# NICTA/revrand

Measured on AMD Instinct MI355X. Metric: feature-rows/sec (Phi + PhiT Phi + PhiT y) at N=10M D=32 F=4096, higher is better.
Workload: dtype f32; 1 GPU; RandomRBF nbases=2048 (F=4096), D=32, N=10000000 f32, features + MFMA Gram, rows sharded over 1 GPU(s); rows_per_gpu=10000000, device=(gfx950:sramecc+:xnack-), gram_engine=f32

## Files before the change

revrand_amd/csrc/rr_rff.hip:

```cpp
#include "rr_syrk_args.h"
#include <algorithm>
#include <map>
#include <mutex>
#include <type_traits>




__device__ __forceinline__ void sincos_rev(float t, float &s, float &c) {
    const float f = t - __builtin_rintf(t);
    s = __builtin_amdgcn_sinf(f);
    c = __builtin_amdgcn_cosf(f);
}

__device__ __forceinline__ void sincos_rev(double t, double &s, double &c) { rr_sincos_rev_f64(t, s, c); }
typedef double doublex4 __attribute__((ext_vector_type(4)));

template <int DMAX, bool GUARD, typename TX, typename TC>
__device__ __forceinline__ TC project_row(const TX *__restrict__ xr, int d, const TC (&w)[DMAX]) {
    TC z = 0;
#pragma unroll
    for (int i = 0; i < DMAX; ++i) {
        if (!GUARD || i < d) z = fma((TC)xr[i], w[i], z);
    }
    return z;
}

template <int DMAX, typename TC>
__device__ __forceinline__ void load_w(TC (&w)[DMAX], const TC *__restrict__ Ws, int npad, int f) {
#pragma unroll
    for (int i = 0; i < DMAX; ++i) w[i] = Ws[(size_t)i * npad + f];
}

constexpr int RR_XS_ROWS = 16;
template <int DMAX, typename TX, typename TC>
__device__ __forceinline__ void stage_x_rows(TC (*xs)[DMAX], const TX *__restrict__ X, int64_t rb, int64_t rvalid, int64_t ldx) {
    for (int e = threadIdx.x; e < RR_XS_ROWS * DMAX; e += 256) {
        const int rr = e / DMAX, i = e % DMAX;
        xs[rr][i] = (rb + rr < rvalid) ? (TC)X[(rb + rr) * ldx + i] : (TC)0;
    }
}
template <int DMAX, typename TC>
__device__ __forceinline__ TC project_lds(const TC *__restrict__ xr, const TC (&w)[DMAX]) {
    TC z0 = 0, z1 = 0, z2 = 0, z3 = 0;
#pragma unroll
    for (int i = 0; i < DMAX; i += 4) {
        z0 = fma(xr[i], w[i], z0);
        z1 = fma(xr[i + 1], w[i + 1], z1);
        z2 = fma(xr[i + 2], w[i + 2], z2);
        z3 = fma(xr[i + 3], w[i + 3], z3);
    }
    return (z0 + z1) + (z2 + z3);
}

template <int DMAX, typename TX, typename TC, typename TO>
__global__ void __launch_bounds__(256)
rr_rff_transform_kernel(const TX *__restrict__ X, int64_t N, int64_t ldx, const TC *__restrict__ Ws,
                        int n, int npad, TO *__restrict__ Phi, int64_t ldphi, TC scale,
                        int rows_per_block) {
    const int f = blockIdx.x * 256 + threadIdx.x;
    const bool fvalid = f < n;
    TC w[DMAX];
    load_w<DMAX, TC>(w, Ws, npad, fvalid ? f : 0);
    const int64_t r0 = (int64_t)blockIdx.y * rows_per_block;
    int64_t r1 = r0 + rows_per_block;
    if (r1 > N) r1 = N;
    if constexpr (sizeof(TC) == 8 && DMAX >= 8) {
        __shared__ TC xs[RR_XS_ROWS][DMAX];
        for (int64_t rb = r0; rb < r1; rb += RR_XS_ROWS) {
            __syncthreads();
            stage_x_rows<DMAX, TX, TC>(xs, X, rb, r1, ldx);
            __syncthreads();
            const int nr = (int)(r1 - rb < RR_XS_ROWS ? r1 - rb : RR_XS_ROWS);
            for (int rr = 0; rr < nr; ++rr) {
                TC s, c;
                sincos_rev(project_lds<DMAX, TC>(xs[rr], w), s, c);
                if (fvalid) {
                    TO *o = Phi + (rb + rr) * ldphi;
                    o[f] = (TO)(c * scale);
                    o[n + f] = (TO)(s * scale);
                }
            }
        }
        return;
    }
    for (int64_t r = r0; r < r1; ++r) {
        const TC t = project_row<DMAX, false, TX, TC>(X + r * ldx, DMAX, w);
// ... 879 lines not shown
            RR_PAIRD(4, o0, o1) RR_PAIRD(5, o1, o0) RR_PAIRD(6, o0, o1) RR_PAIRD(7, o1, o0)
            __syncthreads();
        }
    }

    const int64_t F = p.F;
    const int hi = lane >> 5;
#pragma unroll
    for (int e = 0; e < NB; ++e) {
        const int64_t gc = ca + 32 * bj[e] + (lane & 31);
#pragma unroll
        for (int k = 0; k < 16; ++k) {
            const int64_t gr = ca + 32 * bi[e] + (k & 3) + 8 * (k >> 2) + 4 * hi;
            if (gr <= gc) rr_syrk_out(p, ks, gr, gc, acc[e][k]);
        }
    }
    (void)F;
}
#undef RR_PAIRD

__global__ void __launch_bounds__(GR_THREADS, 2)
rr_syrk_f32_diag_kernel(const SyrkArgs p) {
    __shared__ float lds[2 * GR_KB * GR_TC];
    const int lane = threadIdx.x & 63;
    const int wave = __builtin_amdgcn_readfirstlane(threadIdx.x >> 6);
    if (wave < 4)
        syrk_diag_body<5>(p, lds, wave, lane);
    else
        syrk_diag_body<4>(p, lds, wave, lane);
}

typedef float floatx4 __attribute__((ext_vector_type(4)));

template <int OFF>
__device__ __forceinline__ float lds_read_b32_off(unsigned addr) {
    float r;
    asm volatile("ds_read_b32 %0, %1 offset:%2" : "=v"(r) : "v"(addr), "i"(OFF));
    return r;
}

template <int NB, int ED>
struct KOpsD16 {
    float2v a[NB], b[NB];
    float x0, x1;
    template <int P>
    __device__ __forceinline__ void load(const unsigned (&abase)[NB], const unsigned (&bbase)[NB], unsigned xbase) {
#pragma unroll
        for (int e = 0; e < NB; ++e)
            if (e != ED) a[e] = lds_read2st64<16 * P, 16 * P + 8>(abase[e]);
#pragma unroll
        for (int e = 0; e < NB; ++e)
            if (e != ED) b[e] = lds_read2st64<16 * P, 16 * P + 8>(bbase[e]);
        x0 = lds_read_b32_off<4096 * P>(xbase);
        x1 = lds_read_b32_off<4096 * P + 64>(xbase);
    }
};

template <int NB, int ED, int FIRST, int LAST>
__device__ __forceinline__ void gram_mfma_d16(const KOpsD16<NB, ED> &o, floatx16 (&acc)[NB], floatx4 (&dd)[3]) {
#pragma unroll
    for (int q = FIRST; q < LAST; ++q) {
        if (q < NB - 1 || q >= NB + 2) {
            const int s_ = q < NB - 1 ? 0 : 1;
            const int r_ = q < NB - 1 ? q : q - (NB + 2);
            const int e = r_ < ED ? r_ : r_ + 1;
            acc[e] = __builtin_amdgcn_mfma_f32_32x32x2f32(o.a[e][s_], o.b[e][s_], acc[e], 0, 0, 0);
        } else {
            const int t = q - (NB - 1);
            dd[t] = __builtin_amdgcn_mfma_f32_16x16x4f32(t == 2 ? o.x1 : o.x0, t == 0 ? o.x0 : o.x1, dd[t], 0, 0, 0);
        }
    }
}

#define RR_PAIRD16(P, CUR, NXT)                                \
    lds_wait();                                                \
    __builtin_amdgcn_sched_barrier(0);                         \
    gram_mfma_d16<NB, ED, 0, 1>(CUR, acc, dd);                 \
    __builtin_amdgcn_sched_barrier(0);                         \
    if ((P) + 1 < KB / 4) NXT.template load<((P) + 1) & (KB / 4 - 1)>(abase, bbase, xbase); \
    __builtin_amdgcn_sched_barrier(0);                         \
    gram_mfma_d16<NB, ED, 1, 2 * NB + 1>(CUR, acc, dd);        \
    __builtin_amdgcn_sched_barrier(0);

template <int NB, int ED, int KB>
__device__ __forceinline__ void syrk_diag16_body(const SyrkArgs &p, float *lds, int wave, int lane, const unsigned bid) {
    const int ta = bid % p.nb;
    const int ks = bid / p.nb;
    const int ca = ta * GR_TC;
    const int64_t row_begin = (int64_t)ks * p.rows_per_split;
    int64_t row_end = row_begin + p.rows_per_split;
    if (row_end > p.rows) row_end = p.rows;

    const unsigned lds0 = (unsigned)(size_t)(__attribute__((address_space(3))) float *)lds;
    const unsigned lane_off = 4u * ((lane >> 5) * GR_TC + (lane & 31));
    int bi[NB], bj[NB];
#pragma unroll
    for (int e = 0; e < NB; ++e) {
        bi[e] = RR_DIAG_I[wave][e];
        bj[e] = RR_DIAG_J[wave][e];
    }
    RR_DEV_ASSERT(bi[ED] == bj[ED]);
    const unsigned lane_off16 = 4u * ((lane >> 4) * GR_TC + 32 * bi[ED] + (lane & 15));
    floatx16 acc[NB];
    floatx4 dd[3];
#pragma unroll
    for (int e = 0; e < NB; ++e)
#pragma unroll
        for (int k = 0; k < 16; ++k) acc[e][k] = 0.f;
#pragma unroll
    for (int t = 0; t < 3; ++t) dd[t] = floatx4{0.f, 0.f, 0.f, 0.f};

    const unsigned voff = 16u * lane, ldp4 = (unsigned)p.ldp * 4u;
    auto dma_tile = [&](float *buf, int64_t kb0) {
        RR_DEV_ASSERT(kb0 + KB <= p.rows && ca + GR_TC <= p.ldp && p.rows % KB == 0 && p.rows_per_split % KB == 0);
        const rr_rsrc_t ra = rr_make_rsrc(p.P + kb0 * p.ldp + ca, 0x7fffffffu);
#pragma unroll
        for (int k = 0; k < KB / 8; ++k) {
            const int lr = (KB / 8) * wave + k;
            __builtin_amdgcn_raw_ptr_buffer_load_lds(ra, (lptr_t)(buf + lr * GR_TC), 16, voff, (unsigned)lr * ldp4, 0, 0);
        }
    };

    const int64_t nkb = (row_end - row_begin) / KB;
    if (nkb > 0) {
        dma_tile(lds, row_begin);
        __syncthreads();
        for (int64_t kb = 0; kb < nkb; ++kb) {
            const int cbuf = (int)(kb & 1);
            const int slot = p.spread ? rr_dma_slot(wave, p.spread) : 0;
            auto dma_next = [&]() {
                if (kb + 1 < nkb) dma_tile(lds + (cbuf ^ 1) * (KB * GR_TC), row_begin + (kb + 1) * KB);
            };
            if (slot == 0) dma_next();
            unsigned abase[NB], bbase[NB];
#pragma unroll
            for (int e = 0; e < NB; ++e) {
                abase[e] = lds0 + cbuf * (4u * KB * GR_TC) + lane_off + 128u * bi[e];
                bbase[e] = lds0 + cbuf * (4u * KB * GR_TC) + lane_off + 128u * bj[e];
            }
            const unsigned xbase = lds0 + cbuf * (4u * KB * GR_TC) + lane_off16;
            KOpsD16<NB, ED> o0, o1;
            o0.template load<0>(abase, bbase, xbase);
            RR_PAIRD16(0, o0, o1)
            if (slot == 1) dma_next();
            RR_PAIRD16(1, o1, o0)
            if (slot == 2) dma_next();
            RR_PAIRD16(2, o0, o1)
            if (slot == 3) dma_next();
            RR_PAIRD16(3, o1, o0)
            RR_PAIRD16(4, o0, o1) RR_PAIRD16(5, o1, o0) RR_PAIRD16(6, o0, o1) RR_PAIRD16(7, o1, o0)
            if constexpr (KB == 64) {
                RR_PAIRD16(8, o0, o1) RR_PAIRD16(9, o1, o0) RR_PAIRD16(10, o0, o1) RR_PAIRD16(11, o1, o0)
                RR_PAIRD16(12, o0, o1) RR_PAIRD16(13, o1, o0) RR_PAIRD16(14, o0, o1) RR_PAIRD16(15, o1, o0)
            }
            __syncthreads();
        }
    }

    const int hi = lane >> 5;
#pragma unroll
    for (int e = 0; e < NB; ++e) {
        if (e == ED) continue;
        const int64_t gc = ca + 32 * bj[e] + (lane & 31);
#pragma unroll
        for (int k = 0; k < 16; ++k) {
            const int64_t gr = ca + 32 * bi[e] + (k & 3) + 8 * (k >> 2) + 4 * hi;
            if (gr <= gc) rr_syrk_out(p, ks, gr, gc, acc[e][k]);
        }
    }
#pragma unroll
    for (int t = 0; t < 3; ++t) {
        const int64_t gc = ca + 32 * bi[ED] + (t >= 1 ? 16 : 0) + (lane & 15);
#pragma unroll
        for (int k = 0; k < 4; ++k) {
            const int64_t gr = ca + 32 * bi[ED] + (t == 2 ? 16 : 0) + 4 * (lane >> 4) + k;
            if (gr <= gc) rr_syrk_out(p, ks, gr, gc, dd[t][k]);
        }
    }
}
#undef RR_PAIRD16

template <int KB>
__device__ __forceinline__ void syrk_diag16_dispatch(const SyrkArgs &p, float *lds, const unsigned bid) {
    const int lane = threadIdx.x & 63;
    const int wave = __builtin_amdgcn_readfirstlane(threadIdx.x >> 6);
    switch (wave) {
        case 0: case 1: case 2: case 3: syrk_diag16_body<5, 0, KB>(p, lds, wave, lane, bid); break;
        case 4: syrk_diag16_body<4, 3, KB>(p, lds, wave, lane, bid); break;
        case 5: syrk_diag16_body<4, 2, KB>(p, lds, wave, lane, bid); break;
        case 6: syrk_diag16_body<4, 1, KB>(p, lds, wave, lane, bid); break;
        default: syrk_diag16_body<4, 0, KB>(p, lds, wave, lane, bid); break;
    }
}

template <int KB>
__global__ void __launch_bounds__(GR_THREADS, 2)
rr_syrk_f32_diag16_kernel(const SyrkArgs p) {
    __shared__ float lds[2 * KB * GR_TC];
    syrk_diag16_dispatch<KB>(p, lds, blockIdx.x);
}

constexpr int GS_TC = 128, GS_KB = 32, GS_LD = 2 * GS_TC, GS_THREADS = 256;

__global__ void __launch_bounds__(GS_THREADS, 2)
rr_syrk_f32_small_kernel(const SyrkArgs p) {
    __shared__ __attribute__((aligned(16))) float lds[2][GS_KB * GS_LD];
    const int tid = threadIdx.x, lane = tid & 63, wave = tid >> 6, wr = wave >> 1, wc = wave & 1;
    const int nb = (int)(p.ldp / GS_TC);
    const int64_t ks = blockIdx.x / p.ntiles;
    int t = (int)(blockIdx.x % p.ntiles), ta = 0;
    while (t >= nb - ta) {
        t -= nb - ta;
        ++ta;
    }
    const int tb = ta + t;
    const int64_t ca = (int64_t)ta * GS_TC, cb = (int64_t)tb * GS_TC;
    const int64_t r0 = ks * p.rows_per_split;
    int64_t r1 = r0 + p.rows_per_split;
    if (r1 > p.rows) r1 = p.rows;
    const int nkb = (int)((r1 - r0 + GS_KB - 1) / GS_KB);
    floatx16 acc[2][2];
#pragma unroll
    for (int i = 0; i < 2; ++i)
#pragma unroll
        for (int j = 0; j < 2; ++j)
#pragma unroll
            for (int e = 0; e < 16; ++e) acc[i][j][e] = 0.f;
    const int lr = tid >> 5, lc = tid & 31;
    float4 ra[4], rb[4];
    auto gload = [&](int kb) {
        const float *base = p.P + (r0 + (int64_t)kb * GS_KB + lr) * p.ldp;
#pragma unroll
        for (int u = 0; u < 4; ++u) {
            ra[u] = *(const float4 *)(base + (int64_t)8 * u * p.ldp + ca + 4 * lc);
            rb[u] = *(const float4 *)(base + (int64_t)8 * u * p.ldp + cb + 4 * lc);
        }
    };
    auto lstore = [&](int buf) {
#pragma unroll
        for (int u = 0; u < 4; ++u) {
            *(float4 *)&lds[buf][(lr + 8 * u) * GS_LD + 4 * lc] = ra[u];
            *(float4 *)&lds[buf][(lr + 8 * u) * GS_LD + GS_TC + 4 * lc] = rb[u];
        }
    };
    if (nkb > 0) {
        gload(0);
        lstore(0);
    }
    __syncthreads();
    const int i32 = lane & 31, kk = lane >> 5;
    for (int kb = 0; kb < nkb; ++kb) {
        const int cur = kb & 1;
        if (kb + 1 < nkb) gload(kb + 1);
        const float *L = lds[cur];
#pragma unroll
        for (int k2 = 0; k2 < GS_KB; k2 += 2) {
            const float *row = L + (k2 + kk) * GS_LD;
            const float a0 = row[wr * 64 + i32], a1 = row[wr * 64 + 32 + i32];
            const float b0 = row[GS_TC + wc * 64 + i32], b1 = row[GS_TC + wc * 64 + 32 + i32];
            acc[0][0] = __builtin_amdgcn_mfma_f32_32x32x2f32(a0, b0, acc[0][0], 0, 0, 0);
            acc[0][1] = __builtin_amdgcn_mfma_f32_32x32x2f32(a0, b1, acc[0][1], 0, 0, 0);
            acc[1][0] = __builtin_amdgcn_mfma_f32_32x32x2f32(a1, b0, acc[1][0], 0, 0, 0);
            acc[1][1] = __builtin_amdgcn_mfma_f32_32x32x2f32(a1, b1, acc[1][1], 0, 0, 0);
        }
        if (kb + 1 < nkb) lstore(cur ^ 1);
        __syncthreads();
    }
#pragma unroll
    for (int i = 0; i < 2; ++i)
#pragma unroll
        for (int j = 0; j < 2; ++j) {
            const int64_t gc = cb + wc * 64 + 32 * j + i32;
#pragma unroll
            for (int e = 0; e < 16; ++e) {
                const int64_t gr = ca + wr * 64 + 32 * i + (e & 3) + 8 * (e >> 2) + 4 * kk;
                if (gr <= gc) rr_syrk_out(p, ks, gr, gc, acc[i][j][e]);
            }
        }
}

__global__ void __launch_bounds__(GR_THREADS, 2)
rr_syrk_f32_merged_kernel(const SyrkArgs p, const SyrkArgs pd, const unsigned n_off) {
    __shared__ float lds[2 * GR_KB * GR_LD];
    if (blockIdx.x < n_off) rr_syrk_f32_body<3>(p, lds, blockIdx.x);
    else syrk_diag16_dispatch<32>(pd, lds, blockIdx.x - n_off);
}

constexpr int G64_TC = 128;
constexpr int G64_KB = 16;
constexpr int G64_LDB = 2 * G64_TC * 8 + 128;
constexpr int G64_THREADS = 256;

struct Syrk64Args {
    const double *P;
    int64_t rows, ldp;
    int F, nb, ntiles;
    int64_t rows_per_split;
    double *G;
    int offdiag_only;
    int lower_tri = 0;
    double *part = nullptr;
    int64_t part_stride = 0;
};

__device__ __forceinline__ void rr_syrk64_out(const Syrk64Args &p, int64_t ks, int64_t gr, int64_t gc, double v) {
    if (p.part != nullptr) p.part[ks * p.part_stride + gr * p.ldp + gc] = v;
    else unsafeAtomicAdd(&p.G[gr * (int64_t)p.F + gc], v);
}

template <typename T>
__global__ void __launch_bounds__(256)
rr_syrk_det_reduce_kernel(const T *__restrict__ part, int64_t stride, int64_t ldp, int F, int nsplit, double *__restrict__ G,
                          double *__restrict__ bcol) {
    const int64_t gc = (int64_t)blockIdx.x * 256 + threadIdx.x, gr = blockIdx.y;
    if (gc < gr || gc > F || (gc == F && bcol == nullptr)) return;
    const T *q = part + gr * ldp + gc;
    double s = 0.0;
    for (int k = 0; k < nsplit; ++k) s += (double)q[(int64_t)k * stride];
    if (gc < F) G[gr * (int64_t)F + gc] += s;
    else bcol[gr] += s;
}

template <int OFF>
__device__ __forceinline__ double lds_read_b64(unsigned addr) {
    double r;
    asm volatile("ds_read_b64 %0, %1 offset:%2" : "=v"(r) : "v"(addr), "i"(OFF));
    return r;
}

struct KOps64 {
    double a[4], b[4];
    template <int T>
    __device__ __forceinline__ void load(unsigned abase, unsigned bbase) {
#pragma unroll
        for (int i = 0; i < 4; ++i) a[i] = 0;
        a[0] = lds_read_b64<4 * T * G64_LDB + 0 * 128>(abase);
        a[1] = lds_read_b64<4 * T * G64_LDB + 1 * 128>(abase);
        a[2] = lds_read_b64<4 * T * G64_LDB + 2 * 128>(abase);
        a[3] = lds_read_b64<4 * T * G64_LDB + 3 * 128>(abase);
        b[0] = lds_read_b64<4 * T * G64_LDB + 0 * 128>(bbase);
        b[1] = lds_read_b64<4 * T * G64_LDB + 1 * 128>(bbase);
        b[2] = lds_read_b64<4 * T * G64_LDB + 2 * 128>(bbase);
        b[3] = lds_read_b64<4 * T * G64_LDB + 3 * 128>(bbase);
    }
};

template <int FIRST, int LAST>
__device__ __forceinline__ void gram64_mfma(const KOps64 &o, doublex4 (&acc)[4][4]) {
#pragma unroll
    for (int q = FIRST; q < LAST; ++q)
        acc[q >> 2][q & 3] = __builtin_amdgcn_mfma_f64_16x16x4f64(o.a[q >> 2], o.b[q & 3], acc[q >> 2][q & 3], 0, 0, 0);
}

#define RR_STEP64(T, CUR, NXT)                                  \
    lds_wait();                                                 \
    __builtin_amdgcn_sched_barrier(0);                          \
    gram64_mfma<0, 1>(CUR, acc);                                \
    __builtin_amdgcn_sched_barrier(0);                          \
    if ((T) + 1 < 4) NXT.template load<((T) + 1) & 3>(abase, bbase); \
    __builtin_amdgcn_sched_barrier(0);                          \
    gram64_mfma<1, 16>(CUR, acc);                               \
    __builtin_amdgcn_sched_barrier(0);

__global__ void __launch_bounds__(G64_THREADS, 2)
rr_syrk_f64_kernel(const Syrk64Args p) {
    __shared__ __attribute__((aligned(16))) unsigned char lds[2 * G64_KB * G64_LDB];

    const int tid = threadIdx.x;
// ... 912 lines not shown
            int c2 = 0;
            for (size_t i = 0; i < cnt.size(); ++i) c2 += cnt[i] > 0;
            return c2;
        };
        auto delta_one = [&](int x, int out, int in) {
            int before = 0, after = 0;
            const int bl[4] = {ta[out], tb[out], ta[in], tb[in]};
            for (int i = 0; i < 4; ++i) {
                bool seen = false;
                for (int j = 0; j < i; ++j) seen = seen || bl[j] == bl[i];
                if (seen) continue;
                const int b = bl[i];
                const int c0 = cnt[(size_t)x * nb + b];
                const int c1 = c0 - ((ta[out] == b) || (tb[out] == b) ? 1 : 0) + ((ta[in] == b) || (tb[in] == b) ? 1 : 0);
                before += c0 > 0;
                after += c1 > 0;
            }
            return after - before;
        };
        uint64_t rng = 0x9E3779B97F4A7C15ull;
        auto next = [&]() {
            rng ^= rng << 13; rng ^= rng >> 7; rng ^= rng << 17;
            return rng;
        };
        int cur = cost_of(), best = cur;
        std::vector<int> best_part = part;
        const int64_t iters = std::min<int64_t>((int64_t)20000 * ntiles, 6000000);
        for (int64_t it = 0; it < iters; ++it) {
            const int t1 = (int)(next() % (uint64_t)ntiles), t2 = (int)(next() % (uint64_t)ntiles);
            const int x = part[t1], y = part[t2];
            if (x == y) continue;
            const int d = delta_one(x, t1, t2) + delta_one(y, t2, t1);
            const double temp = 0.4 * (1.0 - (double)it / (double)iters) + 0.05;
            if (d <= 0 || (double)(next() >> 11) / 9007199254740992.0 < exp(-(double)d / temp)) {
                add(x, t1, -1); add(y, t2, -1); add(x, t2, 1); add(y, t1, 1);
                part[t1] = y; part[t2] = x;
                cur += d;
                if (cur < best) { best = cur; best_part = part; }
            }
        }
        part = best_part;
    }
    std::vector<int> fill(nxcd, 0);
    for (int t = 0; t < ntiles; ++t) map[(size_t)fill[part[t]]++ * nxcd + part[t]] = t;
}


int rr_launch_syrk_f32(rr_ctx *c, const float *P, int64_t rows, int64_t ldp, int F, double *dG, hipEvent_t mid,
                       double *bcol = nullptr) {
    if (c->gram_engine != 0) {
        RR_REQUIRE(bcol == nullptr, "gram: the rider column needs the f32 engine");
        RR_REQUIRE(!c->deterministic, "gram: deterministic mode (rr_set_deterministic) needs the f32 engine, not a split 16-bit one");
        return rr_launch_syrk_bf16(c, c->gram_engine, P, nullptr, rows, ldp, F, dG, mid);
    }
    RR_REQUIRE(bcol == nullptr || F < ldp, "gram: no pad column for the rider");
    static const bool small_off = getenv("RR_SYRK_SMALL") != nullptr && atoi(getenv("RR_SYRK_SMALL")) == 0;
    const int64_t big_tiles = (ldp / GR_TC) * (ldp / GR_TC + 1) / 2;
    if (!small_off && ldp <= 1024 && big_tiles * ((rows + 1023) / 1024) < c->num_cu && rows % GS_KB == 0 && !getenv("RR_GRAM_ABLATE")) {
        const int nbs = (int)(ldp / GS_TC), nt = nbs * (nbs + 1) / 2;
        int64_t ns = std::max<int64_t>((2 * c->num_cu + nt - 1) / nt, (rows + 32767) / 32768);
        ns = std::min<int64_t>(ns, std::max<int64_t>(rows / 128, 1));
        const int64_t rps_s = ((rows + ns - 1) / ns + GS_KB - 1) / GS_KB * GS_KB;
        ns = (rows + rps_s - 1) / rps_s;
        SyrkArgs a;
        a.P = P; a.rows = rows; a.ldp = ldp; a.F = F; a.nb = nbs; a.ntiles = nt; a.rows_per_split = rps_s; a.G = dG;
        a.bcol = bcol; a.tile_map = nullptr; a.offdiag_only = 0; a.ablate = 0;
        if (c->deterministic) {
            void *slabs = nullptr;
            int rc = rr_det_scratch(c, (size_t)ns * (size_t)ldp * (size_t)ldp * sizeof(float), &slabs);
            if (rc != RR_OK) return rc;
            a.part = (float *)slabs;
            a.part_stride = ldp * ldp;
        }
        hipLaunchKernelGGL(rr_syrk_f32_small_kernel, dim3((unsigned)(ns * nt)), dim3(GS_THREADS), 0, c->stream, a);
        if (mid) RR_CHECK_HIP(hipEventRecord(mid, c->stream));
        if (a.part)
            hipLaunchKernelGGL(rr_syrk_det_reduce_kernel<float>, dim3((unsigned)((F + 1 + 255) / 256), (unsigned)F), dim3(256), 0,
                               c->stream, a.part, a.part_stride, ldp, F, (int)ns, dG, bcol);
        RR_CHECK_HIP(hipGetLastError());
        return RR_OK;
    }
    const int nb_all = (int)(ldp / GR_TC);
    const int od = (nb_all >= 2 && !getenv("RR_SYRK_NO_DIAG_KERNEL")) ? 1 : 0;
    const int w_last = F + (bcol ? 1 : 0) - GR_TC * (nb_all - 1);
    const int rg = (od && nb_all >= 3 && w_last <= 192 && !getenv("RR_SYRK_NO_RAGGED_KERNEL")) ? 1 : 0;
    const int nb = nb_all - rg;
    const int ntiles = od ? nb * (nb - 1) / 2 : nb * (nb + 1) / 2;
    const int nxcd = 8;
    const bool use_map = (ntiles % nxcd == 0) && !getenv("RR_GRAM_NO_TILE_MAP");
    if (use_map && c->tile_map_nb != nb * 2 + od) {
        std::vector<int> map;
        rr_build_tile_map(nb, od, nxcd, map);
        if (c->tile_map) (void)hipFree(c->tile_map);
        c->tile_map = nullptr;
        RR_CHECK_HIP(hipMalloc((void **)&c->tile_map, map.size() * sizeof(int)));
        RR_CHECK_HIP(hipMemcpy(c->tile_map, map.data(), map.size() * sizeof(int), hipMemcpyHostToDevice));
        c->tile_map_nb = nb * 2 + od;
    }
    const int64_t total_tiles = (int64_t)nb_all * (nb_all + 1) / 2;
    auto gcd64 = [](int64_t x, int64_t y) { while (y) { const int64_t u = x % y; x = y; y = u; } return x; };
    const int64_t min_splits = (rows + 32767) / 32768;
    auto rows_per = [&](int64_t ns) { return ((rows + ns - 1) / ns + GR_KB - 1) / GR_KB * GR_KB; };
    const int64_t unit = ntiles > 0 ? c->num_cu / gcd64(c->num_cu, ntiles) : 1;
    int64_t nsplit = (min_splits + unit - 1) / unit * unit;
    auto floor_rows = [&](int64_t tiles_per_split) {
        return tiles_per_split * ((rows + 1023) / 1024) < c->num_cu ? (int64_t)256 : (int64_t)1024;
    };
    auto small_split = [&](int64_t tiles_per_split) {
        const int64_t fr = floor_rows(tiles_per_split);
        if (fr == 1024) return (rows + 1023) / 1024;
        const int64_t want = (c->num_cu + tiles_per_split - 1) / std::max<int64_t>(tiles_per_split, 1);
        return std::min((rows + fr - 1) / fr, std::max((rows + 1023) / 1024, want));
    };
    if (rows / nsplit < 1024) {
        nsplit = small_split(std::max(ntiles, 1));
        static const bool no_search = getenv("RR_SYRK_SPLIT_SEARCH") != nullptr && atoi(getenv("RR_SYRK_SPLIT_SEARCH")) == 0;
        if (ntiles > 0 && !no_search) {
            double best_cost = 1e300;
            int64_t best_ns = nsplit;
            const int64_t ns_hi = std::max<int64_t>(rows / 256, 1), ns_lo = std::max<int64_t>(rows / 32768, 1);
            for (int64_t ns = ns_lo; ns <= ns_hi && ns <= ns_lo + 4096; ++ns) {
                const int64_t rp = rows_per(ns), n2 = (rows + rp - 1) / rp;
                const int64_t rounds = ((int64_t)ntiles * n2 + c->num_cu - 1) / c->num_cu;
                const double cost = (double)rounds * ((double)rp + 96.0);
                if (cost < best_cost - 1e-9) {
                    best_cost = cost;
                    best_ns = n2;
                }
            }
            nsplit = best_ns;
        }
    }
    if (nsplit < 1) nsplit = 1;
    int64_t rps = rows_per(nsplit);
    int64_t nsplit_d = nsplit, rps_d = rps;
    if (od) {
        double best = -1.0;
        for (int64_t ns = min_splits; ns < min_splits + 96; ++ns) {
            if (rows / ns < floor_rows(nb_all) && ns > 1) break;
            const int64_t wg = ns * nb_all, rounds = (wg + c->num_cu - 1) / c->num_cu;
            const double eff = (double)wg / (double)(rounds * c->num_cu);
            if (eff > best + 1e-9) {
                best = eff;
                nsplit_d = ns;
            }
        }
        rps_d = rows_per(nsplit_d);
        if (rows % 64 == 0 && getenv("RR_SYRK_DIAG_KB") != nullptr && atoi(getenv("RR_SYRK_DIAG_KB")) == 64)
            rps_d = (rps_d + 63) / 64 * 64;
    }
    int64_t nsplit_r = nsplit, rps_r = rps;
    if (rg) {
        double best = -1.0;
        for (int64_t ns = min_splits; ns < min_splits + 96; ++ns) {
            if (rows / ns < floor_rows(nb_all - 1) && ns > 1) break;
            const int64_t wg = ns * (nb_all - 1), rounds = (wg + c->num_cu - 1) / c->num_cu;
            const double eff = (double)wg / (double)(rounds * c->num_cu);
            if (eff > best + 1e-9) {
                best = eff;
                nsplit_r = ns;
            }
        }
        rps_r = rows_per(nsplit_r);
    }
    const char *renv = getenv("RR_GRAM_ROWS_PER_SPLIT");
    if (renv && atoll(renv) >= GR_KB) rps = rps_d = rps_r = (atoll(renv) / GR_KB) * GR_KB;
    if (c->deterministic) rps_d = rps_r = rps;
    nsplit = (rows + rps - 1) / rps;
    nsplit_d = (rows + rps_d - 1) / rps_d;
    nsplit_r = (rows + rps_r - 1) / rps_r;
    RR_REQUIRE(nsplit * total_tiles < (int64_t)1 << 31 && nsplit_d * nb_all < (int64_t)1 << 31 &&
                   nsplit_r * nb_all < (int64_t)1 << 31, "gram: grid too large");
    SyrkArgs a;
    a.P = P; a.rows = rows; a.ldp = ldp; a.F = F; a.nb = nb; a.ntiles = ntiles; a.rows_per_split = rps; a.G = dG;
    a.bcol = bcol;
    a.tile_map = use_map ? c->tile_map : nullptr;
    a.offdiag_only = od;
    a.ablate = getenv("RR_GRAM_ABLATE") ? atoi(getenv("RR_GRAM_ABLATE")) : 0;
    a.spread = rr_dma_spread_env();
    if (c->deterministic) {
        void *slabs = nullptr;
        int rc = rr_det_scratch(c, (size_t)nsplit * (size_t)ldp * (size_t)ldp * sizeof(float), &slabs);
        if (rc != RR_OK) return rc;
        a.part = (float *)slabs;
        a.part_stride = ldp * ldp;
    }
    static const int syrk_mode = getenv("RR_SYRK_STAGGER") ? atoi(getenv("RR_SYRK_STAGGER")) : 3;
    static const bool merge_diag = getenv("RR_SYRK_MERGE_DIAG") != nullptr && atoi(getenv("RR_SYRK_MERGE_DIAG")) != 0;
    if (merge_diag && od && !rg && ntiles > 0 && syrk_mode == 3 && !a.ablate && !getenv("RR_SYRK_NO_DIAG16")) {
        SyrkArgs ad = a;
        ad.nb = nb_all;
        ad.rows_per_split = rps_d;
        const unsigned n_off = (unsigned)(nsplit * ntiles);
        hipLaunchKernelGGL(rr_syrk_f32_merged_kernel, dim3(n_off + (unsigned)(nsplit_d * nb_all)), dim3(GR_THREADS), 0, c->stream, a, ad, n_off);
        if (mid) RR_CHECK_HIP(hipEventRecord(mid, c->stream));
        if (a.part)
            hipLaunchKernelGGL(rr_syrk_det_reduce_kernel<float>, dim3((unsigned)((F + 1 + 255) / 256), (unsigned)F), dim3(256), 0,
                               c->stream, a.part, a.part_stride, ldp, F, (int)nsplit, dG, bcol);
        RR_CHECK_HIP(hipGetLastError());
        return RR_OK;
    }
    if (ntiles > 0) {
        if (syrk_mode == 1 && !a.ablate)
            hipLaunchKernelGGL(rr_syrk_f32_flatstag_kernel, dim3((unsigned)(nsplit * ntiles)), dim3(GR_THREADS), 0, c->stream, a);
        else if (syrk_mode == 2 && !a.ablate)
            hipLaunchKernelGGL(rr_syrk_f32_buf_kernel, dim3((unsigned)(nsplit * ntiles)), dim3(GR_THREADS), 0, c->stream, a);
        else if (syrk_mode == 0 || a.ablate)
            hipLaunchKernelGGL(rr_syrk_f32_flat_kernel, dim3((unsigned)(nsplit * ntiles)), dim3(GR_THREADS), 0, c->stream, a);
        else
            hipLaunchKernelGGL(rr_syrk_f32_kernel, dim3((unsigned)(nsplit * ntiles)), dim3(GR_THREADS), 0, c->stream, a);
    }
    if (rg) {
        SyrkArgs ar = a;
        ar.nb = nb_all;
        ar.rows_per_split = rps_r;
        hipLaunchKernelGGL(rr_syrk_f32_ragged_kernel, dim3((unsigned)(nsplit_r * (nb_all - 1))), dim3(GR_THREADS), 0, c->stream, ar);
    }
    if (mid) RR_CHECK_HIP(hipEventRecord(mid, c->stream));
    if (od) {
        SyrkArgs ad = a;
        ad.nb = nb_all;
        ad.rows_per_split = rps_d;
        static const bool no_diag16 = getenv("RR_SYRK_NO_DIAG16") != nullptr;
        static const bool kb64 = getenv("RR_SYRK_DIAG_KB") != nullptr && atoi(getenv("RR_SYRK_DIAG_KB")) == 64;
        if (no_diag16)
            hipLaunchKernelGGL(rr_syrk_f32_diag_kernel, dim3((unsigned)(nsplit_d * nb_all)), dim3(GR_THREADS), 0, c->stream, ad);
        else if (kb64 && rows % 64 == 0 && ad.rows_per_split % 64 == 0)
            hipLaunchKernelGGL(rr_syrk_f32_diag16_kernel<64>, dim3((unsigned)(nsplit_d * nb_all)), dim3(GR_THREADS), 0, c->stream, ad);
        else
            hipLaunchKernelGGL(rr_syrk_f32_diag16_kernel<32>, dim3((unsigned)(nsplit_d * nb_all)), dim3(GR_THREADS), 0, c->stream, ad);
    }
    if (a.part)
        hipLaunchKernelGGL(rr_syrk_det_reduce_kernel<float>, dim3((unsigned)((F + 1 + 255) / 256), (unsigned)F), dim3(256), 0,
                           c->stream, a.part, a.part_stride, ldp, F, (int)nsplit, dG, bcol);
    RR_CHECK_HIP(hipGetLastError());
    return RR_OK;
}

int rr_launch_syrk_f64(rr_ctx *c, const double *P, int64_t rows, int64_t ldp, int F, double *dG, int lower_tri = 0) {
    const int nb = (int)(ldp / G64_TC);
    const int od = (nb >= 2 && !getenv("RR_SYRK_NO_DIAG_KERNEL")) ? 1 : 0;
    const int ntiles = od ? nb * (nb - 1) / 2 : nb * (nb + 1) / 2;
    const int64_t slots = (int64_t)c->num_cu * 2;
    int64_t g = slots, t = ntiles;
    while (t) { const int64_t u = g % t; g = t; t = u; }
    const int64_t unit = slots / g;
    static const bool no_fine = getenv("RR_SYRK64_FINE_SPLIT") != nullptr && atoi(getenv("RR_SYRK64_FINE_SPLIT")) == 0;
    const int64_t min_rows = (lower_tri && rows == ldp && rows <= 2048 && !no_fine) ? 128 : 512;
    int64_t nsplit = unit;
    if (rows / nsplit < 2048) nsplit = (slots * 4 + ntiles - 1) / ntiles;
    if (rows / nsplit < min_rows) nsplit = (rows + min_rows - 1) / min_rows;
    if (nsplit < 1) nsplit = 1;
    const int64_t rps = ((rows + nsplit - 1) / nsplit + G64_KB - 1) / G64_KB * G64_KB;
    nsplit = (rows + rps - 1) / rps;
    RR_REQUIRE(nsplit * ntiles < (int64_t)1 << 31, "gram: grid too large");
    Syrk64Args a;
    a.P = P; a.rows = rows; a.ldp = ldp; a.F = F; a.nb = nb; a.ntiles = ntiles; a.rows_per_split = rps; a.G = dG;
    a.offdiag_only = od;
    static const bool no_tri = getenv("RR_SYRK64_TRI") != nullptr && atoi(getenv("RR_SYRK64_TRI")) == 0;
    a.lower_tri = lower_tri && !no_tri && rows == ldp ? 1 : 0;
    if (c->deterministic) {
        void *slabs = nullptr;
        int rc = rr_det_scratch(c, (size_t)nsplit * (size_t)ldp * (size_t)ldp * sizeof(double), &slabs);
        if (rc != RR_OK) return rc;
        a.part = (double *)slabs;
        a.part_stride = ldp * ldp;
    }
    if (ntiles > 0)
        hipLaunchKernelGGL(rr_syrk_f64_kernel, dim3((unsigned)(nsplit * ntiles)), dim3(G64_THREADS), 0, c->stream, a);
    if (od) {
        const int64_t dslots = (int64_t)c->num_cu * 4;
        int64_t best_ns = 1;
        double best = -1.0;
        for (int64_t ns = 1; ns <= 4 * dslots / nb + 1; ++ns) {
            if (rows / ns < min_rows && ns > 1) break;
            const int64_t wg = ns * nb, rounds = (wg + dslots - 1) / dslots;
            const double eff = (double)wg / (double)(rounds * dslots);
            if (eff > best + 1e-9) {
                best = eff;
                best_ns = ns;
            }
        }
        Syrk64Args ad = a;
        ad.rows_per_split = ((rows + best_ns - 1) / best_ns + G64_KB - 1) / G64_KB * G64_KB;
        if (c->deterministic) ad.rows_per_split = rps;
        const int64_t nsd = (rows + ad.rows_per_split - 1) / ad.rows_per_split;
        hipLaunchKernelGGL(rr_syrk_f64_diag_kernel, dim3((unsigned)(nsd * nb)), dim3(G64_THREADS), 0, c->stream, ad);
    }
    if (a.part)
        hipLaunchKernelGGL(rr_syrk_det_reduce_kernel<double>, dim3((unsigned)((F + 255) / 256), (unsigned)F), dim3(256), 0,
                           c->stream, a.part, a.part_stride, ldp, F, (int)nsplit, dG, (double *)nullptr);
    RR_CHECK_HIP(hipGetLastError());
    return RR_OK;
}

int rr_launch_gemm_tn_f64(rr_ctx *c, const double *A, int64_t lda, const double *B, int64_t ldb, double *D, int64_t ldd,
                          int64_t K, int64_t M, int64_t N, int subtract, int upper_only) {
    Gemm64Args g;
    g.A = A; g.B = B; g.D = D; g.lda = lda; g.ldb = ldb; g.ldd = ldd; g.K = (int)K; g.ntb = (int)(N / G64_TC);
    g.subtract = subtract;
    g.upper_only = upper_only;
    static const bool no_k128 = getenv("RR_GEMM64_K128") != nullptr && atoi(getenv("RR_GEMM64_K128")) == 0;
    if (!no_k128 && K == 128 && M == 128 && N % 32 == 0 && (upper_only == 0 || (upper_only == 1 && N == 128))) {
        hipLaunchKernelGGL(rr_gemm_tn_f64_k128_kernel, dim3((unsigned)(N / 32)), dim3(G64_THREADS), 0, c->stream, g);
        RR_CHECK_HIP(hipGetLastError());
        return RR_OK;
    }
    hipLaunchKernelGGL(rr_gemm_tn_f64_kernel, dim3((unsigned)((M / G64_TC) * g.ntb)), dim3(G64_THREADS), 0, c->stream, g);
    RR_CHECK_HIP(hipGetLastError());
    return RR_OK;
}

template <typename TX, typename TC>
// ... 858 lines not shown
```

Before: 8.418 million feature-rows/s.

## Rewrite diagonal SYRK tile kernel with 4 waves dealing 9 blocks each

The default diagonal-tile Gram kernel now runs 256 threads (4 waves) per workgroup instead of 8 waves. Each wave takes 9 of the 36 upper 32x32 blocks, two of them diagonal blocks done with 16x16 MFMAs, and loads only the LDS columns its blocks need, tracked through a compile-time column mask. The split-count search now counts two workgroup slots per CU, and the old 8-wave kernel stays available behind an env flag. The KB=64 variant and the merged off-diagonal/diagonal launch are removed, so each wave does more work and keeps more accumulators in registers.

```diff
diff --git a/revrand_amd/csrc/rr_rff.hip b/revrand_amd/csrc/rr_rff.hip
--- a/revrand_amd/csrc/rr_rff.hip
+++ b/revrand_amd/csrc/rr_rff.hip
@@ -3,6 +3,7 @@
 #include <map>
 #include <mutex>
 #include <type_traits>
+#include <utility>
 
 
 
@@ -1048,8 +1049,9 @@
     gram_mfma_d16<NB, ED, 1, 2 * NB + 1>(CUR, acc, dd);        \
     __builtin_amdgcn_sched_barrier(0);
 
-template <int NB, int ED, int KB>
+template <int NB, int ED>
 __device__ __forceinline__ void syrk_diag16_body(const SyrkArgs &p, float *lds, int wave, int lane, const unsigned bid) {
+    constexpr int KB = GR_KB;
     const int ta = bid % p.nb;
     const int ks = bid / p.nb;
     const int ca = ta * GR_TC;
@@ -1115,10 +1117,6 @@
             if (slot == 3) dma_next();
             RR_PAIRD16(3, o1, o0)
             RR_PAIRD16(4, o0, o1) RR_PAIRD16(5, o1, o0) RR_PAIRD16(6, o0, o1) RR_PAIRD16(7, o1, o0)
-            if constexpr (KB == 64) {
-                RR_PAIRD16(8, o0, o1) RR_PAIRD16(9, o1, o0) RR_PAIRD16(10, o0, o1) RR_PAIRD16(11, o1, o0)
-                RR_PAIRD16(12, o0, o1) RR_PAIRD16(13, o1, o0) RR_PAIRD16(14, o0, o1) RR_PAIRD16(15, o1, o0)
-            }
             __syncthreads();
         }
     }
@@ -1146,24 +1144,212 @@
 }
 #undef RR_PAIRD16
 
-template <int KB>
-__device__ __forceinline__ void syrk_diag16_dispatch(const SyrkArgs &p, float *lds, const unsigned bid) {
+__global__ void __launch_bounds__(GR_THREADS, 2)
+rr_syrk_f32_diag16_wg8_kernel(const SyrkArgs p) {
+    __shared__ float lds[2 * GR_KB * GR_TC];
     const int lane = threadIdx.x & 63;
     const int wave = __builtin_amdgcn_readfirstlane(threadIdx.x >> 6);
     switch (wave) {
-        case 0: case 1: case 2: case 3: syrk_diag16_body<5, 0, KB>(p, lds, wave, lane, bid); break;
-        case 4: syrk_diag16_body<4, 3, KB>(p, lds, wave, lane, bid); break;
-        case 5: syrk_diag16_body<4, 2, KB>(p, lds, wave, lane, bid); break;
-        case 6: syrk_diag16_body<4, 1, KB>(p, lds, wave, lane, bid); break;
-        default: syrk_diag16_body<4, 0, KB>(p, lds, wave, lane, bid); break;
-    }
-}
+        case 0: case 1: case 2: case 3: syrk_diag16_body<5, 0>(p, lds, wave, lane, blockIdx.x); break;
+        case 4: syrk_diag16_body<4, 3>(p, lds, wave, lane, blockIdx.x); break;
+        case 5: syrk_diag16_body<4, 2>(p, lds, wave, lane, blockIdx.x); break;
+        case 6: syrk_diag16_body<4, 1>(p, lds, wave, lane, blockIdx.x); break;
+        default: syrk_diag16_body<4, 0>(p, lds, wave, lane, blockIdx.x); break;
+    }
+}
+
+constexpr int GD_THREADS = 256, GD_NBLK = 9;
+constexpr int RR_DIAG4_I[4][GD_NBLK] = {{0, 1, 0, 0, 0, 0, 1, 1, 1}, {2, 3, 2, 2, 3, 0, 1, 2, 3},
+                                        {4, 5, 4, 4, 4, 5, 5, 3, 3}, {6, 7, 6, 0, 0, 1, 1, 2, 2}};
+constexpr int RR_DIAG4_J[4][GD_NBLK] = {{0, 1, 1, 2, 3, 4, 2, 3, 4}, {2, 3, 3, 4, 4, 5, 5, 5, 5},
+                                        {4, 5, 5, 6, 7, 6, 7, 6, 7}, {6, 7, 7, 6, 7, 6, 7, 6, 7}};
+constexpr bool rr_diag4_deal_ok() {
+    int seen[8][8] = {};
+    for (int w = 0; w < 4; ++w)
+        for (int e = 0; e < GD_NBLK; ++e) {
+            const int i = RR_DIAG4_I[w][e], j = RR_DIAG4_J[w][e];
+            if (i < 0 || j > 7 || i > j || (e < 2) != (i == j)) return false;
+            ++seen[i][j];
+        }
+    for (int i = 0; i < 8; ++i)
+        for (int j = 0; j < 8; ++j)
+            if (seen[i][j] != (i <= j ? 1 : 0)) return false;
+    return true;
+}
+static_assert(rr_diag4_deal_ok(), "diagonal tile: the 36 upper blocks, 9 per wave, each exactly once");
+
+template <int W>
+struct RrDiag4 {
+    static constexpr int ND = 2, NF = GD_NBLK - ND, NQ = 2 * NF + 3 * ND;
+    static constexpr int bi(int n) { return RR_DIAG4_I[W][ND + n]; }
+    static constexpr int bj(int n) { return RR_DIAG4_J[W][ND + n]; }
+    static constexpr unsigned mask() {
+        unsigned m = 0;
+        for (int n = 0; n < NF; ++n) m |= (1u << bi(n)) | (1u << bj(n));
+        return m;
+    }
+    static constexpr int popc(unsigned m) { int c = 0; for (; m; m &= m - 1) ++c; return c; }
+    static constexpr int NOP = popc(mask());
+    static constexpr int op(int col) { return popc(mask() & ((1u << col) - 1u)); }
+    static constexpr int col(int slot) {
+        for (int c = 0; c < 8; ++c)
+            if (((mask() >> c) & 1u) && op(c) == slot) return c;
+        return -1;
+    }
+};
+
+template <int B, int... I, typename Fn>
+__device__ __forceinline__ void rr_static_for_impl(std::integer_sequence<int, I...>, Fn &&f) {
+    (f(std::integral_constant<int, B + I>{}), ...);
+}
+template <int B, int E, typename Fn>
+__device__ __forceinline__ void rr_static_for(Fn &&f) {
+    if constexpr (E > B) rr_static_for_impl<B>(std::make_integer_sequence<int, E - B>{}, f);
+}
+
+template <typename D>
+struct KOpsD4 {
+    float2v c[D::NOP];
+    float x0[D::ND], x1[D::ND];
+    template <int P>
+    __device__ __forceinline__ void load(const unsigned (&cbase)[D::NOP], const unsigned (&xbase)[D::ND]) {
+#pragma unroll
+        for (int n = 0; n < D::NOP; ++n) c[n] = lds_read2st64<16 * P, 16 * P + 8>(cbase[n]);
+#pragma unroll
+        for (int n = 0; n < D::ND; ++n) {
+            x0[n] = lds_read_b32_off<4096 * P>(xbase[n]);
+            x1[n] = lds_read_b32_off<4096 * P + 64>(xbase[n]);
+        }
+    }
+};
+
+template <typename D, int FIRST, int LAST>
+__device__ __forceinline__ void gram_mfma_d4(const KOpsD4<D> &o, floatx16 (&acc)[D::NF], floatx4 (&dd)[3 * D::ND]) {
+    rr_static_for<FIRST, LAST>([&](auto qc) __attribute__((always_inline)) {
+        constexpr int q = decltype(qc)::value;
+        if constexpr (q < D::NF || q >= D::NF + 3 * D::ND) {
+            constexpr int s_ = q < D::NF ? 0 : 1;
+            constexpr int n = q < D::NF ? q : q - (D::NF + 3 * D::ND), oa = D::op(D::bi(n)), ob = D::op(D::bj(n));
+            acc[n] = __builtin_amdgcn_mfma_f32_32x32x2f32(o.c[oa][s_], o.c[ob][s_], acc[n], 0, 0, 0);
+        } else {
+            constexpr int t = q - D::NF, n = t / 3, u = t % 3;
+            dd[t] = __builtin_amdgcn_mfma_f32_16x16x4f32(u == 2 ? o.x1[n] : o.x0[n], u == 0 ? o.x0[n] : o.x1[n], dd[t], 0, 0, 0);
+        }
+    });
+}
+
+#define RR_PAIRD4(P, CUR, NXT)                                 \
+    lds_wait();                                                \
+    __builtin_amdgcn_sched_barrier(0);                         \
+    gram_mfma_d4<D, 0, 1>(CUR, acc, dd);                       \
+    __builtin_amdgcn_sched_barrier(0);                         \
+    if ((P) + 1 < 8) NXT.template load<((P) + 1) & 7>(cbase, xbase); \
+    __builtin_amdgcn_sched_barrier(0);                         \
+    gram_mfma_d4<D, 1, D::NQ>(CUR, acc, dd);                   \
+    __builtin_amdgcn_sched_barrier(0);
+
+template <int W>
+__device__ __forceinline__ void syrk_diag4_body(const SyrkArgs &p, float *lds, int lane) {
+    using D = RrDiag4<W>;
+    const int ta = blockIdx.x % p.nb;
+    const int ks = blockIdx.x / p.nb;
+    const int ca = ta * GR_TC;
+    const int64_t row_begin = (int64_t)ks * p.rows_per_split;
+    int64_t row_end = row_begin + p.rows_per_split;
+    if (row_end > p.rows) row_end = p.rows;
+
+    const unsigned lds0 = (unsigned)(size_t)(__attribute__((address_space(3))) float *)lds;
+    const unsigned lane_off = 4u * ((lane >> 5) * GR_TC + (lane & 31));
+    const unsigned lane_off16 = 4u * ((lane >> 4) * GR_TC + (lane & 15));
+    floatx16 acc[D::NF];
+    floatx4 dd[3 * D::ND];
+#pragma unroll
+    for (int n = 0; n < D::NF; ++n)
+#pragma unroll
+        for (int k = 0; k < 16; ++k) acc[n][k] = 0.f;
+#pragma unroll
+    for (int t = 0; t < 3 * D::ND; ++t) dd[t] = floatx4{0.f, 0.f, 0.f, 0.f};
+
+    const unsigned voff = 16u * lane, ldp4 = (unsigned)p.ldp * 4u;
+    auto dma_tile = [&](float *buf, int64_t kb0) {
+        RR_DEV_ASSERT(kb0 + GR_KB <= p.rows && ca + GR_TC <= p.ldp && p.rows % GR_KB == 0 && p.rows_per_split % GR_KB == 0);
+        const rr_rsrc_t ra = rr_make_rsrc(p.P + kb0 * p.ldp + ca, 0x7fffffffu);
+#pragma unroll
+        for (int k = 0; k < GR_KB / 4; ++k) {
+            const int lr = (GR_KB / 4) * W + k;
+            __builtin_amdgcn_raw_ptr_buffer_load_lds(ra, (lptr_t)(buf + lr * GR_TC), 16, voff, (unsigned)lr * ldp4, 0, 0);
+        }
+    };
+
+    const int64_t nkb = (row_end - row_begin) / GR_KB;
+    if (nkb > 0) {
+        dma_tile(lds, row_begin);
+        __syncthreads();
+        const int slot = p.spread ? rr_dma_slot(W, p.spread) : 0;
+        for (int64_t kb = 0; kb < nkb; ++kb) {
+            const int cbuf = (int)(kb & 1);
+            auto dma_next = [&]() {
+                if (kb + 1 < nkb) dma_tile(lds + (cbuf ^ 1) * (GR_KB * GR_TC), row_begin + (kb + 1) * GR_KB);
+            };
+            if (slot == 0) dma_next();
+            const unsigned cur = lds0 + cbuf * (4u * GR_KB * GR_TC);
+            unsigned cbase[D::NOP], xbase[D::ND];
+            rr_static_for<0, D::NOP>([&](auto nc) __attribute__((always_inline)) {
+                constexpr int n = decltype(nc)::value, col = D::col(n);
+                cbase[n] = cur + lane_off + 128u * col;
+            });
+            rr_static_for<0, D::ND>([&](auto nc) __attribute__((always_inline)) {
+                constexpr int n = decltype(nc)::value, blk = RR_DIAG4_I[W][n];
+                xbase[n] = cur + lane_off16 + 128u * blk;
+            });
+            KOpsD4<D> o0, o1;
+            o0.template load<0>(cbase, xbase);
+            RR_PAIRD4(0, o0, o1)
+            if (slot == 1) dma_next();
+            RR_PAIRD4(1, o1, o0)
+            if (slot == 2) dma_next();
+            RR_PAIRD4(2, o0, o1)
+            if (slot == 3) dma_next();
+            RR_PAIRD4(3, o1, o0)
+            RR_PAIRD4(4, o0, o1) RR_PAIRD4(5, o1, o0) RR_PAIRD4(6, o0, o1) RR_PAIRD4(7, o1, o0)
+            __syncthreads();
+        }
+    }
+
+    const int hi = lane >> 5;
+    rr_static_for<0, D::NF>([&](auto nc) __attribute__((always_inline)) {
+        constexpr int n = decltype(nc)::value, bi = D::bi(n), bj = D::bj(n);
+        const int64_t gc = ca + 32 * bj + (lane & 31);
+#pragma unroll
+        for (int k = 0; k < 16; ++k) {
+            const int64_t gr = ca + 32 * bi + (k & 3) + 8 * (k >> 2) + 4 * hi;
+            if (gr <= gc) rr_syrk_out(p, ks, gr, gc, acc[n][k]);
+        }
+    });
+    rr_static_for<0, 3 * D::ND>([&](auto tc) __attribute__((always_inline)) {
+        constexpr int t = decltype(tc)::value, n = t / 3, u = t % 3, blk = RR_DIAG4_I[W][n];
+        const int64_t gc = ca + 32 * blk + (u >= 1 ? 16 : 0) + (lane & 15);
+#pragma unroll
+        for (int k = 0; k < 4; ++k) {
+            const int64_t gr = ca + 32 * blk + (u == 2 ? 16 : 0) + 4 * (lane >> 4) + k;
+            if (gr <= gc) rr_syrk_out(p, ks, gr, gc, dd[t][k]);
+        }
+    });
+}
+#undef RR_PAIRD4
 
 template <int KB>
-__global__ void __launch_bounds__(GR_THREADS, 2)
+__global__ void __launch_bounds__(GD_THREADS, 2)
 rr_syrk_f32_diag16_kernel(const SyrkArgs p) {
-    __shared__ float lds[2 * KB * GR_TC];
-    syrk_diag16_dispatch<KB>(p, lds, blockIdx.x);
+    static_assert(KB == GR_KB, "k-blocks of 32 rows");
+    __shared__ float lds[2 * GR_KB * GR_TC];
+    const int lane = threadIdx.x & 63;
+    switch (__builtin_amdgcn_readfirstlane(threadIdx.x >> 6)) {
+        case 0: syrk_diag4_body<0>(p, lds, lane); break;
+        case 1: syrk_diag4_body<1>(p, lds, lane); break;
+        case 2: syrk_diag4_body<2>(p, lds, lane); break;
+        default: syrk_diag4_body<3>(p, lds, lane); break;
+    }
 }
 
 constexpr int GS_TC = 128, GS_KB = 32, GS_LD = 2 * GS_TC, GS_THREADS = 256;
@@ -1243,13 +1429,6 @@
                 if (gr <= gc) rr_syrk_out(p, ks, gr, gc, acc[i][j][e]);
             }
         }
-}
-
-__global__ void __launch_bounds__(GR_THREADS, 2)
-rr_syrk_f32_merged_kernel(const SyrkArgs p, const SyrkArgs pd, const unsigned n_off) {
-    __shared__ float lds[2 * GR_KB * GR_LD];
-    if (blockIdx.x < n_off) rr_syrk_f32_body<3>(p, lds, blockIdx.x);
-    else syrk_diag16_dispatch<32>(pd, lds, blockIdx.x - n_off);
 }
 
 constexpr int G64_TC = 128;
@@ -2328,6 +2507,8 @@
     }
     const int nb_all = (int)(ldp / GR_TC);
     const int od = (nb_all >= 2 && !getenv("RR_SYRK_NO_DIAG_KERNEL")) ? 1 : 0;
+    const char *wg8_env = getenv("RR_SYRK_DIAG_WG8");
+    const bool diag_wg8 = wg8_env != nullptr && atoi(wg8_env) != 0;
     const int w_last = F + (bcol ? 1 : 0) - GR_TC * (nb_all - 1);
     const int rg = (od && nb_all >= 3 && w_last <= 192 && !getenv("RR_SYRK_NO_RAGGED_KERNEL")) ? 1 : 0;
     const int nb = nb_all - rg;
@@ -2382,18 +2563,17 @@
     int64_t nsplit_d = nsplit, rps_d = rps;
     if (od) {
         double best = -1.0;
+        const int64_t slots = diag_wg8 ? c->num_cu : 2 * c->num_cu;
         for (int64_t ns = min_splits; ns < min_splits + 96; ++ns) {
             if (rows / ns < floor_rows(nb_all) && ns > 1) break;
-            const int64_t wg = ns * nb_all, rounds = (wg + c->num_cu - 1) / c->num_cu;
-            const double eff = (double)wg / (double)(rounds * c->num_cu);
+            const int64_t wg = ns * nb_all, rounds = (wg + slots - 1) / slots;
+            const double eff = (double)wg / (double)(rounds * slots);
             if (eff > best + 1e-9) {
                 best = eff;
                 nsplit_d = ns;
             }
         }
         rps_d = rows_per(nsplit_d);
-        if (rows % 64 == 0 && getenv("RR_SYRK_DIAG_KB") != nullptr && atoi(getenv("RR_SYRK_DIAG_KB")) == 64)
-            rps_d = (rps_d + 63) / 64 * 64;
     }
     int64_t nsplit_r = nsplit, rps_r = rps;
     if (rg) {
@@ -2432,20 +2612,6 @@
         a.part_stride = ldp * ldp;
     }
     static const int syrk_mode = getenv("RR_SYRK_STAGGER") ? atoi(getenv("RR_SYRK_STAGGER")) : 3;
-    static const bool merge_diag = getenv("RR_SYRK_MERGE_DIAG") != nullptr && atoi(getenv("RR_SYRK_MERGE_DIAG")) != 0;
-    if (merge_diag && od && !rg && ntiles > 0 && syrk_mode == 3 && !a.ablate && !getenv("RR_SYRK_NO_DIAG16")) {
-        SyrkArgs ad = a;
-        ad.nb = nb_all;
-        ad.rows_per_split = rps_d;
-        const unsigned n_off = (unsigned)(nsplit * ntiles);
-        hipLaunchKernelGGL(rr_syrk_f32_merged_kernel, dim3(n_off + (unsigned)(nsplit_d * nb_all)), dim3(GR_THREADS), 0, c->stream, a, ad, n_off);
-        if (mid) RR_CHECK_HIP(hipEventRecord(mid, c->stream));
-        if (a.part)
-            hipLaunchKernelGGL(rr_syrk_det_reduce_kernel<float>, dim3((unsigned)((F + 1 + 255) / 256), (unsigned)F), dim3(256), 0,
-                               c->stream, a.part, a.part_stride, ldp, F, (int)nsplit, dG, bcol);
-        RR_CHECK_HIP(hipGetLastError());
-        return RR_OK;
-    }
     if (ntiles > 0) {
         if (syrk_mode == 1 && !a.ablate)
             hipLaunchKernelGGL(rr_syrk_f32_flatstag_kernel, dim3((unsigned)(nsplit * ntiles)), dim3(GR_THREADS), 0, c->stream, a);
@@ -2468,13 +2634,12 @@
         ad.nb = nb_all;
         ad.rows_per_split = rps_d;
         static const bool no_diag16 = getenv("RR_SYRK_NO_DIAG16") != nullptr;
-        static const bool kb64 = getenv("RR_SYRK_DIAG_KB") != nullptr && atoi(getenv("RR_SYRK_DIAG_KB")) == 64;
         if (no_diag16)
             hipLaunchKernelGGL(rr_syrk_f32_diag_kernel, dim3((unsigned)(nsplit_d * nb_all)), dim3(GR_THREADS), 0, c->stream, ad);
-        else if (kb64 && rows % 64 == 0 && ad.rows_per_split % 64 == 0)
-            hipLaunchKernelGGL(rr_syrk_f32_diag16_kernel<64>, dim3((unsigned)(nsplit_d * nb_all)), dim3(GR_THREADS), 0, c->stream, ad);
+        else if (diag_wg8)
+            hipLaunchKernelGGL(rr_syrk_f32_diag16_wg8_kernel, dim3((unsigned)(nsplit_d * nb_all)), dim3(GR_THREADS), 0, c->stream, ad);
         else
-            hipLaunchKernelGGL(rr_syrk_f32_diag16_kernel<32>, dim3((unsigned)(nsplit_d * nb_all)), dim3(GR_THREADS), 0, c->stream, ad);
+            hipLaunchKernelGGL(rr_syrk_f32_diag16_kernel<GR_KB>, dim3((unsigned)(nsplit_d * nb_all)), dim3(GD_THREADS), 0, c->stream, ad);
     }
     if (a.part)
         hipLaunchKernelGGL(rr_syrk_det_reduce_kernel<float>, dim3((unsigned)((F + 1 + 255) / 256), (unsigned)F), dim3(256), 0,
```

New measurement: 8.432 million feature-rows/s, median of 6. Within noise of the previous version (+0.2%).
